# twndus/YelpRecommendation

Measured on AMD Instinct MI355X. Metric: BPR triplets/sec @ dim64, higher is better.
Workload: dtype f32; 1 GPU; BPR-MF dim=64 train step (gather+score+loss+grad+dense Adam), synthetic Yelp2018 shape; users=31668, items=38048, interactions=1566260, train_triplets_per_epoch=920629, batch_per_gpu=524288, global_batch=524288, optimizer=adam(dense), parallelism=single

## Files before the change

### include/yelprec_engine.h

```cpp
#ifndef YELPREC_ENGINE_H
#define YELPREC_ENGINE_H

#include <stdint.h>

#ifdef __cplusplus
extern "C" {
#endif

#define YR_ENGINE_VERSION 36

#define YR_ERR_UNSUPPORTED (-1)
#define YR_ERR_BADARG      (-2)

#define YR_FLAG_BAD_USER 1
#define YR_FLAG_BAD_ITEM 2

#define YR_PULL_USER_PHASE 1
#define YR_PULL_ITEM_PHASE 2

#define YR_S3REC_TRAIN 0
#define YR_S3REC_VALID 1
#define YR_S3REC_TEST  2

#define YR_OPT_ADAM  0
// ... 13 lines not shown
                float *out, int32_t *err_flag, void *stream);

int yr_mf_score_backward(const float *U, const float *I,
                         const int64_t *user, const int64_t *item, const float *gout,
                         int64_t B, int D, int64_t num_users, int64_t num_items,
                         float *gradU, float *gradI, int32_t *err_flag, void *stream);

int yr_bpr_mf_fwd_bwd(const float *U, const float *I,
                      const int64_t *user, const int64_t *pos, const int64_t *neg,
                      int64_t B, int D, int64_t num_users, int64_t num_items,
                      float inv_batch, float *gradU, float *gradI,
                      float *loss_partials, int32_t *err_flag, void *stream);

int yr_bpr_mf_scatter_step(float *U, float *I, float *gradU, float *gradI,
                           float *mU, float *vU, float *mI, float *vI, uint8_t *touched,
                           const int64_t *user, const int64_t *pos, const int64_t *neg,
                           int64_t B, int D, int64_t num_users, int64_t num_items, float inv_batch,
                           double lr, double step_size, double bc2_sqrt,
                           double beta1, double beta2, double eps, double weight_decay, int mode,
                           float *loss_partials, float *loss_out, double *loss_accum,
                           int32_t *err_flag, void *stream);
int yr_adam_dense_dual(float *p0, float *g0, float *m0, float *v0, int64_t n0,
                       float *p1, float *g1, float *m1, float *v1, int64_t n1,
                       int row_width, uint8_t *touched0, uint8_t *touched1,
                       double lr, double step_size, double bc2_sqrt,
                       double beta1, double beta2, double eps, double weight_decay, int mode,
                       const float *loss_partials, float loss_scale, float *loss_out, double *loss_accum,
                       void *stream);

int64_t yr_bpr_mf_pull_workspace_bytes(int64_t max_batch, int64_t num_users, int64_t num_items, int D);
int yr_bpr_mf_pull_step(const float *U_old, float *U_new, float *I,
                        float *mU, float *vU, float *mI, float *vI, float *gradI_out,
                        const int64_t *user, const int64_t *pos, const int64_t *neg,
                        int64_t B, int D, int64_t num_users, int64_t num_items, float inv_batch,
                        double lr, double step_size, double bc2_sqrt,
                        double beta1, double beta2, double eps, double weight_decay, int mode,
                        int deterministic, void *workspace, int64_t workspace_bytes,
                        float *loss_partials, float *loss_out, double *loss_accum,
                        int32_t *err_flag, void *stream);

int yr_bpr_mf_pull_index(const int64_t *user, const int64_t *pos, const int64_t *neg, int64_t B, int D,
                         int64_t num_users, int64_t num_items,
                         void *workspace, int64_t workspace_bytes, int32_t *err_flag, void *stream);
int yr_bpr_mf_pull_apply(const float *U_old, float *U_new, float *I,
                         float *mU, float *vU, float *mI, float *vI, float *gradI_out,
                         int64_t B, int D, int64_t num_users, int64_t num_items, float inv_batch,
                         double lr, double step_size, double bc2_sqrt,
                         double beta1, double beta2, double eps, double weight_decay, int mode,
                         int deterministic, void *workspace, int64_t workspace_bytes,
                         float *loss_partials, float *loss_out, double *loss_accum,
                         int phases, int64_t item_row_begin, int64_t item_row_end,
                         void *stream);
int yr_bpr_mf_pull_item_buckets(int64_t num_items, int D);
int yr_bpr_mf_pull_split_summary(const void *workspace, int64_t workspace_bytes, int64_t B, int D,
                                 int64_t num_users, int64_t num_items, int32_t *counters_out,
                                 int32_t *parts_out, int32_t *rule_out, void *stream);
int yr_bpr_mf_pull_apply_ordered(const float *U_old, float *U_new, float *I,
                         float *mU, float *vU, float *mI, float *vI, float *gradI_out,
                         int64_t B, int D, int64_t num_users, int64_t num_items, float inv_batch,
                         double lr, double step_size, double bc2_sqrt,
                         double beta1, double beta2, double eps, double weight_decay, int mode,
                         int deterministic, void *workspace, int64_t workspace_bytes,
                         float *loss_partials, float *loss_out, double *loss_accum,
                         int phases, int64_t item_row_begin, int64_t item_row_end,
                         const int32_t *item_bucket_order, void *stream);

#define YR_NGCF_MAX_LAYERS 8
int yr_ngcf_score_fwd(const float *const *layers, int n_layers, const int64_t *user, const int64_t *pos,
                      const int64_t *neg, int64_t B, int D, int64_t num_users, int64_t num_items,
                      float *out_pos, float *out_neg, int32_t *err_flag, void *stream);
int yr_ngcf_score_bwd(const float *const *layers, float *const *dlayers, int n_layers, const int64_t *user,
                      const int64_t *pos, const int64_t *neg, const float *gpos, const float *gneg,
                      int64_t B, int D, int64_t num_users, int64_t num_items, int32_t *err_flag, void *stream);
int yr_spmm_csr(const int32_t *rowptr, const int32_t *col, const float *val,
                const float *X, float *Y, int64_t n, int D, int accumulate,
                const int32_t *heavy_rows, int64_t n_heavy, int heavy_threshold, void *stream);
int yr_spmm_csr_sliced(const int32_t *rowptr, const int32_t *col, const float *val,
                       const float *X, float *Y, int64_t n, int D, int accumulate,
                       const int32_t *row_order, void *stream);
int yr_ngcf_dense_fwd(const float *E, const float *Z, const float *W1, const float *W2,
                      int64_t n, int D, float *Eout, void *stream);
int yr_ngcf_dense_bwd_data(const float *dEout, const float *Eout, const float *E, const float *Z,
                           const float *W1T, const float *W2T, int64_t n, int D,
                           float *dZ, float *dE, void *stream);
int yr_ngcf_dense_bwd_weight(const float *dEout, const float *Eout, const float *E, const float *Z,
                             int64_t n, int D, float *dW1, float *dW2, void *stream);

int yr_ngcf_frontier_mark(const int64_t *user, const int64_t *pos, const int64_t *neg, int64_t B,
                          int64_t num_users, int64_t num_items,
                          int32_t *flags, int32_t *rows, int32_t *count, int clear, void *stream);
int yr_ngcf_frontier_expand(const int32_t *rowptr, const int32_t *col, int64_t n,
                            const int32_t *rows_in, const int32_t *count_in, int64_t max_rows_in,
                            int32_t *flags, int32_t *rows, int32_t *count, int clear, void *stream);
int yr_spmm_csr_subset(const int32_t *rowptr, const int32_t *col, const float *val,
                       const float *X, float *Y, int64_t n, int D, int accumulate,
                       const int32_t *heavy_rows, int64_t n_heavy, int heavy_threshold,
                       const int32_t *row_active,
                       const int32_t *row_list, const int32_t *row_count, int64_t max_rows, void *stream);
int yr_spmm_csr_push_rows(const int32_t *rowptr, const int32_t *col, const float *val,
                          const float *X, float *Y, int64_t n, int D,
                          const int32_t *rows, const int32_t *count, int64_t max_rows, void *stream);
int yr_ngcf_dense_fwd_rows(const float *E, const float *Z, const float *W1, const float *W2,
                           int64_t n, int D, float *Eout,
                           const int32_t *rows, const int32_t *count, int64_t max_rows, float *zero_rows,
                           void *stream);
int yr_ngcf_dense_bwd_data_rows(const float *dEout, const float *Eout, const float *E, const float *Z,
// ... 266 lines not shown
```

### yelprecommendation_amd/_lib.py

```python
from __future__ import annotations

import ctypes as C
import os

_HERE = os.path.dirname(os.path.abspath(__file__))
LIB_PATH = os.environ.get("YR_ENGINE_LIB") or os.path.join(_HERE, "libyelprec_engine.so")
ENGINE_VERSION = 36

_p = C.c_void_p
_i64 = C.c_int64
_int = C.c_int
_f = C.c_float
_d = C.c_double

SIGNATURES = {
    "yr_engine_version": [],
    "yr_engine_arch": [],
    "yr_mf_score": [_p, _p, _p, _p, _i64, _int, _i64, _i64, _p, _p, _p],
    "yr_mf_score_backward": [_p, _p, _p, _p, _p, _i64, _int, _i64, _i64, _p, _p, _p, _p],
    "yr_bpr_mf_fwd_bwd": [_p, _p, _p, _p, _p, _i64, _int, _i64, _i64, _f, _p, _p, _p, _p, _p],
    "yr_bpr_mf_scatter_step": [_p, _p, _p, _p, _p, _p, _p, _p, _p, _p, _p, _p, _i64, _int, _i64, _i64, _f,
                               _d, _d, _d, _d, _d, _d, _d, _int, _p, _p, _p, _p, _p],
    "yr_adam_dense_dual": [_p, _p, _p, _p, _i64, _p, _p, _p, _p, _i64, _int, _p, _p,
                           _d, _d, _d, _d, _d, _d, _d, _int, _p, _f, _p, _p, _p],
# ... 4 lines not shown
    "yr_spmm_csr_sliced": [_p, _p, _p, _p, _p, _i64, _int, _int, _p, _p],
    "yr_ngcf_score_fwd": [_p, _int, _p, _p, _p, _i64, _int, _i64, _i64, _p, _p, _p, _p],
    "yr_ngcf_score_bwd": [_p, _p, _int, _p, _p, _p, _p, _p, _i64, _int, _i64, _i64, _p, _p],
    "yr_ngcf_dense_fwd": [_p, _p, _p, _p, _i64, _int, _p, _p],
    "yr_ngcf_dense_bwd_data": [_p, _p, _p, _p, _p, _p, _i64, _int, _p, _p, _p],
    "yr_ngcf_dense_bwd_weight": [_p, _p, _p, _p, _i64, _int, _p, _p, _p],
    "yr_ngcf_frontier_mark": [_p, _p, _p, _i64, _i64, _i64, _p, _p, _p, _int, _p],
    "yr_ngcf_frontier_expand": [_p, _p, _i64, _p, _p, _i64, _p, _p, _p, _int, _p],
    "yr_spmm_csr_subset": [_p, _p, _p, _p, _p, _i64, _int, _int, _p, _i64, _int, _p, _p, _p, _i64, _p],
    "yr_spmm_csr_push_rows": [_p, _p, _p, _p, _p, _i64, _int, _p, _p, _i64, _p],
    "yr_ngcf_dense_fwd_rows": [_p, _p, _p, _p, _i64, _int, _p, _p, _p, _i64, _p, _p],
    "yr_ngcf_dense_bwd_data_rows": [_p, _p, _p, _p, _p, _p, _i64, _int, _p, _p, _p, _p, _i64, _p],
    "yr_ngcf_dense_bwd_weight_rows": [_p, _p, _p, _p, _i64, _int, _p, _p, _p, _p, _i64, _p],
    "yr_ngcf_step_workspace_bytes": [_i64, _int, _int, _i64],
    "yr_ngcf_bpr_step": [_p, _p, _p, _i64, _i64, _p, _i64, _int, _i64, _p, _p, _p, _int, _int, _p, _p, _p, _i64,
                         _d, _d, _d, _d, _d, _d, _d, _int, _d, _p, _i64, _p, _p, _p, _p],
    "yr_ngcf_owned_score_workspace_bytes": [_i64, _i64],
    "yr_ngcf_owned_score_bwd": [_p, _p, _int, _p, _p, _p, _p, _p, _i64, _int, _i64, _i64, _p, _i64, _p, _p],
    "yr_ngcf_owned_dw_workspace_bytes": [_i64, _int],
    "yr_ngcf_owned_dense_bwd_weight": [_p, _p, _p, _p, _i64, _int, _p, _p, _p, _p, _i64, _p, _i64, _p],
    "yr_ngcf_frontier_order": [_p, _i64, _p, _p, _p],
    "yr_ngcf_step_ordered_workspace_bytes": [_i64, _int, _int, _i64],
    "yr_ngcf_bpr_step_ordered": [_p, _p, _p, _i64, _i64, _p, _i64, _int, _i64, _p, _p, _p, _int, _int, _p, _p, _p,
                                 _i64, _d, _d, _d, _d, _d, _d, _d, _int, _d, _p, _i64, _p, _p, _p, _p],
    "yr_gemm_f32": [_int, _int, _i64, _i64, _i64, _p, _i64, _p, _i64, _p, _i64, _p, _int, _int, _int, _p],
    "yr_gemm_f32_ex": [_int, _int, _i64, _i64, _i64, _p, _i64, _p, _i64, _p, _i64, _p, _int, _int, _int, _p, _p, _p],
    "yr_cdae_decode_loss_partials": [_i64, _i64],
    "yr_cdae_decode_loss": [_p, _p, _p, _p, _p, _i64, _i64, _int, _int, _p, _i64, _p, _p, _p, _p],
    "yr_cdae_hidden_bwd": [_p, _p, _int, _p, _i64, _int, _i64, _p, _p, _p, _p, _i64, _p, _p, _p, _int, _p],
    "yr_cdae_compact_pair": [_p, _p, _i64, _i64, C.c_uint64, _d, _p, _p, _p, _p, _p, _p, _p],
    "yr_cdae_train_lists": [_p, _p, _p, _p, _p, _i64, _i64, _i64, _int, C.c_uint64, C.c_uint64, _d, _p, _p, _p, _p, _p,
                            _p, _p, _p],
    "yr_cdae_train_lists_batched": [_p, _p, _p, _p, _p, _i64, _i64, _i64, _int, _p, _p, _i64, _d, _p, _p, _p, _p, _p,
                                    _p, _p, _p],
    "yr_cdae_loss_finalize_batched": [_p, _int, _p, _i64, _i64, _p, _p, _p, _p],
    "yr_cdae_loss_finalize": [_p, _i64, _p, _p, _p, _p],
    "yr_cdae_sampled_decode_splits": [_i64],
    "yr_cdae_sampled_decode": [_p, _p, _p, _p, _p, _p, _i64, _i64, _int, _int, _p, _p, _p, _p, _p, _p],
    "yr_cdae_hidden_init": [_p, _p, _p, _p, _i64, _int, _i64, _p, _p],
    "yr_dropout": [_p, _p, _d, _i64, _p, _p],
    "yr_sigmoid": [_p, _i64, _p],
    "yr_dropout_seeded": [_p, C.c_uint64, _d, _i64, _p, _p],
    "yr_sigmoid_bwd": [_p, _p, _p, _i64, _p],
    "yr_colsum": [_p, _i64, _i64, _p, _int, _p],
    "yr_row_scatter_add": [_p, _p, _i64, _int, _i64, _p, _p],
    "yr_nsbce_fwd": [_p, _p, _p, _i64, _p, _p, _p],
    "yr_nsbce_bwd": [_p, _p, _p, _p, _p, _i64, _p, _p],
    "yr_bpr_mf_pull_index": [_p, _p, _p, _i64, _int, _i64, _i64, _p, _i64, _p, _p],
    "yr_bpr_mf_pull_apply": [_p, _p, _p, _p, _p, _p, _p, _p, _i64, _int, _i64, _i64, _f,
                             _d, _d, _d, _d, _d, _d, _d, _int, _int, _p, _i64, _p, _p, _p, _int, _i64, _i64, _p],
    "yr_bpr_mf_pull_apply_ordered": [_p, _p, _p, _p, _p, _p, _p, _p, _i64, _int, _i64, _i64, _f,
                             _d, _d, _d, _d, _d, _d, _d, _int, _int, _p, _i64, _p, _p, _p, _int, _i64, _i64, _p, _p],
    "yr_bpr_mf_pull_item_buckets": [_i64, _int],
    "yr_bpr_mf_pull_split_summary": [_p, _i64, _i64, _int, _i64, _i64, _p, _p, _p, _p],
    "yr_loss_finalize": [_p, _f, _p, _p, _p],
    "yr_mf_scores_gemm": [_p, _p, _p, _i64, _int, _i64, _i64, _p, _i64, _p, _p],
    "yr_mf_eval_topk_planes_bytes": [_i64, _int],
    "yr_mf_eval_topk_workspace_bytes": [_i64, _i64, _int, _int, _int],
    "yr_mf_eval_topk": [_p, _p, _p, _i64, _int, _i64, _i64, _p, _p, _f, _int, _p, _p, _i64, _int, _p, _p, _p],
    "yr_mf_eval_topk_bias": [_p, _p, _p, _p, _i64, _int, _i64, _i64, _p, _p, _f, _int, _p, _p, _i64, _int, _p, _p, _p],
    "yr_ngcf_eval_topk_workspace_bytes": [_i64, _i64, _int, _int, _int],
    "yr_ngcf_eval_topk": [_p, _int, _int, _p, _i64, _i64, _i64, _p, _p, _f, _int, _p, _p, _i64, _p, _p, _p],
    "yr_topk_masked": [_p, _i64, _i64, _i64, _p, _p, _p, _f, _int, _p, _p],
    "yr_rank_metrics_workspace_bytes": [_i64],
    "yr_rank_metrics": [_p, _i64, _int, _p, _p, _p, _p, _p, _p],
    "yr_bpr_loss_fwd": [_p, _p, _i64, _p, _p],
    "yr_bpr_loss_bwd": [_p, _p, _p, _f, _i64, _p, _p, _p],
    "yr_adam_dense": [_p, _p, _p, _p, _i64, _d, _d, _d, _d, _d, _d, _d, _int, _int, _p],
    "yr_adam_dense_flat": [_p, _p, _p, _p, _p, _p, _p, _p, _p, _p, _int, _d, _d, _d, _d, _d, _d, _d, _int, _p],
    "yr_csr_rows_to_dense": [_p, _p, _p, _i64, _i64, _i64, _int, _p, _p, _p],
    "yr_negative_mask": [_p, _i64, _i64, _int, C.c_uint64, _p, _p, _p],
    "yr_sgd_dense": [_p, _p, _i64, _d, _d, _int, _p],
    "yr_cdae_sparse_part_columns": [_i64],
    "yr_cdae_compact_rows": [_p, _i64, _i64, C.c_uint64, _d, _p, _p, _p, _p],
    "yr_cdae_sparse_encode": [_p, _p, _p, _p, _p, _p, _p, _i64, _i64, _int, _i64, _int, _p, _p, _p],
    "yr_cdae_sparse_dwh": [_p, _p, _p, _p, _i64, _i64, _int, _p, _p, _p, C.c_int32, _p, _p, _p],
    "yr_cdae_sparse_encode_t": [_p, _p, _p, _p, _p, _p, _p, _i64, _i64, _int, _i64, _int, _p, _p, _p],
    "yr_cdae_sparse_dwh_t": [_p, _p, _p, _p, _i64, _i64, _int, _p, _p, _p],
    "yr_cdae_hidden_bwd_dwh_t": [_p, _p, _p, _p, _p, _int, _int, _p, _p, _i64, _i64, _int, _i64, _p, _p, _p, _p, _p, _p,
                                 _i64, _p, _p, _p],
    "yr_cdae_catalogue_bce_workspace_floats": [_i64, _i64, _int],
    "yr_cdae_catalogue_bce": [_p, _p, _p, _p, _p, _p, _i64, _i64, _i64, _int, _int, _p, _p, _p, _p, _p, _i64, _p, _p],
    "yr_cdae_owned_workspace_bytes": [_i64, _i64, _int],
    "yr_cdae_owned_decode": [_p, _p, _p, _p, _p, _p, _i64, _i64, _int, _int, _p, _p, _p, _p, _p, _p, _i64, _p],
    "yr_cdae_owned_hidden_bwd": [_p, _p, _p, _p, _p, _int, _int, _p, _p, _i64, _i64, _int, _i64, _p, _p, _p, _p, _p, _p,
                                 _i64, _p, _p, _p, _i64, _p],
    "yr_triplet_sample": [_p, _p, _i64, _p, _p, _i64, _i64, C.c_uint64, C.c_uint64, _int, _i64, _i64,
                          _p, _p, _p, _p, _p],
    "yr_dcn_assemble": [_p, _p, _p, _p, _p, _p, _int, _int, _i64, _i64, _i64, _i64, _p, _p, _p, _i64, _int, _p, _i64,
                        _p, _p],
    "yr_dcn_assemble_bwd": [_p, _i64, _p, _p, _int, _int, _i64, _i64, _i64, _i64, _p, _p, _p, _i64, _int, _p, _p, _p,
                            _p, _p, _p],
    "yr_relu_bwd": [_p, _p, _i64, _p],
    "yr_dcn_head": [_p, _i64, _p, _i64, _i64, _int, _int, _int, _p, _p, _p, _p, _int, _f, _p, _p, _p, _i64, _p, _i64,
                    _p, _p, _p, _p, _p, _p],
    "yr_dcn_score": [_p, _i64, _p, _i64, _p, _p, _p, _i64, _i64, _i64, _int, _int, _p, _p, _p, _p, _p, _p, _int, _int,
                     _p, _i64, _p, _p],
    "yr_s3rec_encode": [_p, _p, _p, _p, _i64, _int, _int, _int, _int, _i64, _int, _p, _p, _p],
    "yr_s3rec_seq_scores": [_p, _p, _p, _p, _i64, _int, _i64, _p, _p, _p, _p],
    "yr_s3rec_candidate_scores": [_p, _p, _p, _p, _i64, _i64, _int, _i64, _p, _p, _p, _p],
    "yr_s3rec_train_workspace_floats": [_i64, _int, _int, _int, _int],
    "yr_s3rec_encode_train": [_p, _p, _p, _p, _i64, _int, _int, _int, _int, _i64, C.c_uint64, _d, _p, _p, _i64, _p, _p],
    "yr_s3rec_backward": [_p, _p, _p, _i64, _int, _int, _int, _int, C.c_uint64, _d, _p, _i64, _p, _p],
    "yr_s3rec_score_grad": [_p, _p, _p, _p, _p, _i64, _int, _i64, _p, _p, _p],
    "yr_s3rec_item_grad": [_p, _p, _p, _p, _p, _p, _i64, _int, _i64, _p, _p, _p, _p],
    "yr_s3rec_catalogue_bce_workspace_floats": [_i64, _i64, _int],
# ... 61 lines not shown
```

### yelprecommendation_amd/bpr_step.py

```python
import torch

from . import engine
from .user_shard import ItemSlices, reduce_scatter_item_exchange, sharded_item_exchange


AUTO_PULL_MIN_BATCH = 24576

IMPL_NAMES = {
    "auto": "auto: atomic scatter + one Adam launch below %d triplets per rank and step, pull above" % AUTO_PULL_MIN_BATCH,
    "pull": "pull: tile partition + owner pass per table (gather/score/loss/grad/Adam fused, no atomics)",
    "atomic": "atomic: fused gather/score/loss + float-atomic scatter-add, dense Adam",
}


class BPRMFStep:
    def __init__(self, U, I, lr=1e-4, betas=(0.9, 0.999), eps=1e-8, weight_decay=0.0, optimizer="adam",
                 world_size=1, process_group=None, time_kernels=False, impl="auto", max_batch=0,
                 state=None, split_item_update=False, item_chunks=1, item_exchange="all_reduce", rank=0,
                 deterministic=False):
        if item_exchange not in ("all_reduce", "reduce_scatter"):
            raise ValueError("item_exchange must be 'all_reduce' or 'reduce_scatter'")
        width = int(U.shape[1])
        if width in engine.WIDE_WIDTHS:
            limit = max(engine.SUPPORTED_WIDTHS)
# ... 89 lines not shown
                                              self.U.device)
            self._ws_slots[slot], self._ws_batch[slot] = ws, batch
        return ws

    def step(self, u, p, n, record=False, global_batch=None, next_batch=None):
        if global_batch is None:
            global_batch = u.numel() * self.world_size
        key = self.impl_key
        if key == "auto":
            key = "pull" if (global_batch >= AUTO_PULL_MIN_BATCH * self.world_size and self._pull_ok) else "atomic"
            if self._slices is not None or self.deterministic:
                key = "pull"
        if key == "pull":
            if self._U_alt is None:
                self._U_alt = torch.empty_like(self.U)
            self.impl = IMPL_NAMES["pull"]
            self.launches = "tile_partition, owner_pass<user>, owner_pass<item>"
            return self._step_pull(u, p, n, record, global_batch, next_batch)
        if self.gU is None:
            self.gU = torch.zeros_like(self.U)
        if self.gI is None:
            self.gI = torch.zeros_like(self.I)
        self.impl = IMPL_NAMES["atomic"]
        self.launches = "bpr_fwd_bwd, adam_dual"
        return self._step_atomic(u, p, n, record, global_batch)

    def _check_triplets(self, u, p, n):
        B = u.numel()
        for name, t in (("user", u), ("pos", p), ("neg", n)):
            if not (t.is_cuda and t.dtype == torch.int64 and t.is_contiguous() and t.numel() == B):
                raise engine.EngineError(f"{name}: need a contiguous int64 GPU tensor of length {B}")
        return B

    def _build_index(self, u, p, n, slot):
        B = self._check_triplets(u, p, n)
        ws = self._workspace(B, slot)
        rc = self._lib.yr_bpr_mf_pull_index(u.data_ptr(), p.data_ptr(), n.data_ptr(), B, self.U.shape[1],
                                            self.U.shape[0], self.I.shape[0], ws.data_ptr(), ws.numel(),
                                            self._pflag, engine._stream())
        if rc:
            engine.check(rc, "yr_bpr_mf_pull_index")
        self._indexed = (slot, (u, p, n))

    def set_item_order(self, item_weight=None):
        if item_weight is None:
            self._item_order = None
            return
        nb = int(self._lib.yr_bpr_mf_pull_item_buckets(self.I.shape[0], self.I.shape[1]))
        rows = -(-self.I.shape[0] // nb) if nb else 1
        per = 1024 // self.I.shape[1]
        w = torch.zeros(nb * per, dtype=torch.float64, device=self.I.device)
        w[:self.I.shape[0]] = item_weight.to(self.I.device, torch.float64)
        load = w.view(nb, per).sum(1)
        self._item_order = torch.argsort(load, descending=True, stable=True).to(torch.int32).contiguous()

    def _auto_item_order(self, p, n):
        rows = self.I.shape[0]
        ids = torch.cat([p, n])
        ids = ids[(ids >= 0) & (ids < rows)]
        self.set_item_order(torch.bincount(ids, minlength=rows)[:rows])

    def _step_pull(self, u, p, n, record, global_batch, next_batch=None):
        B = u.numel()
        D = self.U.shape[1]
        if self._item_order is None and self.auto_item_order and B >= 4 * self.I.shape[0]:
            self._auto_item_order(p, n)
        inv = 1.0 / global_batch if global_batch else 0.0
        self.t += 1
        multi = self.world_size > 1 or self.split_item_update
        nU, nI = self.U.numel(), self.I.numel()
        alg = B * (24 + 24 * D) + 6 * 4 * (nU + (0 if multi else nI))
        ready = self._indexed is not None and all(a is b for a, b in zip(self._indexed[1], (u, p, n)))
        slot = self._indexed[0] if ready else 0

        nchunks = self.item_chunks if multi else 1
        rows = self.I.shape[0]
        gran = engine.pull_bucket_rows(D)
        bounds = [min(rows, (rows * c // nchunks + gran - 1) // gran * gran) for c in range(nchunks)] + [rows]
        both = engine.PULL_USER_PHASE | engine.PULL_ITEM_PHASE
        ploss, paccum = self.loss.data_ptr(), self.loss_accum.data_ptr()

        def apply(phases, r0, r1, with_loss=None):
            ws = self._ws_slots[slot]
            if with_loss is None:
                with_loss = bool(phases & engine.PULL_USER_PHASE)
            step_size, bc2_sqrt = engine.adam_scalars(self.t, self.lr, self.betas[0], self.betas[1])
            order = self._item_order
            rc = self._lib.yr_bpr_mf_pull_apply_ordered(
                self.U.data_ptr(), self._U_alt.data_ptr(), self._pI, self._pmU, self._pvU, self._pmI, self._pvI,
                self.gI.data_ptr() if multi else None, B, D, self.U.shape[0], rows, inv, self.lr,
                step_size, bc2_sqrt, self.betas[0], self.betas[1], self.eps, self.wd,
                engine.OPT_ADAMW if self.decoupled else engine.OPT_ADAM, 1 if self.deterministic else 0,
                ws.data_ptr(), ws.numel(), self._ppartials, ploss if with_loss else None,
                paccum if with_loss else None, phases, r0, r1, order.data_ptr() if order is not None else None,
                engine._stream())
            if rc:
                engine.check(rc, "yr_bpr_mf_pull_apply_ordered")

        def first_chunk():
            if not ready:
                self._build_index(u, p, n, slot)
            apply(both, bounds[0], bounds[1])
            if nchunks == 1:
                self._indexed = None

        def local_first():
            if record and self.time_kernels and not multi and self.t % 2 == 0:
# ... 123 lines not shown
```

### yelprecommendation_amd/csrc/bpr_pull.hip

```cpp
#include "adam.h"
#include "common.h"

namespace yr {

constexpr int kPartThreads = 1024;
#ifndef YR_ITEM_CAP
#define YR_ITEM_CAP 1024
#endif
constexpr int kCap = YR_ITEM_CAP;
constexpr int kUserCap = 768;
constexpr int kTileGroup = 256;
constexpr int kOccShift = 26;
constexpr int kOccMask = (1 << kOccShift) - 1;
constexpr int kMaxBuckets = 16383;
constexpr int kMaxOwnerGrid = 4096;
#ifndef YR_HEAVY_ROW
#define YR_HEAVY_ROW 96
#endif
constexpr int kHeavyRow = YR_HEAVY_ROW;
#ifndef YR_SPLIT_MIN
#define YR_SPLIT_MIN 2048
#endif
constexpr int kSplitMin = YR_SPLIT_MIN;
#ifndef YR_SPLIT_AVG_MIN
#define YR_SPLIT_AVG_MIN 2.5
#endif
#ifndef YR_SPLIT_AVG_TARGET
#define YR_SPLIT_AVG_TARGET 1.25
#endif
#ifndef YR_SPLIT_TARGET
#define YR_SPLIT_TARGET 1024
#endif
constexpr int kSplitTarget = YR_SPLIT_TARGET;
constexpr int kMaxParts = 64;
constexpr int kMaxTasks = 512;
constexpr int kMaxSlots = 1024;
#ifndef YR_ROWSPLIT
#define YR_ROWSPLIT 1
#endif
#ifndef YR_ROWSPLIT_MIN
#define YR_ROWSPLIT_MIN 1024
#endif
#ifndef YR_ROWSPLIT_AVG_MIN
#define YR_ROWSPLIT_AVG_MIN 2.32
#endif
#ifndef YR_ROWSPLIT_TARGET
#define YR_ROWSPLIT_TARGET 512
#endif
#ifndef YR_ROWSPLIT_AVG_TARGET
#define YR_ROWSPLIT_AVG_TARGET 1.16
#endif
constexpr int kRowSplitMin = YR_ROWSPLIT_MIN;
constexpr int kRowSplitTarget = YR_ROWSPLIT_TARGET;
constexpr int kMaxRowTasks = YR_ROWSPLIT ? 512 : 0;
constexpr int kBuildLanes = 4;
#ifndef YR_DEAL
#define YR_DEAL 1
#endif
#ifndef YR_DEAL_MIN
#define YR_DEAL_MIN 256
#endif
constexpr int kDealMin = YR_DEAL_MIN;
#ifndef YR_OWNER_WAVES
#define YR_OWNER_WAVES 8
#endif
#ifndef YR_USER_UNROLL
#define YR_USER_UNROLL 1
#endif
#ifndef YR_ITEM_UNROLL
#define YR_ITEM_UNROLL 2
#endif
constexpr int kUserUnroll = YR_USER_UNROLL;
constexpr int kItemUnroll = YR_ITEM_UNROLL;

struct PullAdam {
  AdamScalars c;
  int decoupled;
};

__device__ __forceinline__ float4 ld4o(const float* base, uint32_t off) {
  return *reinterpret_cast<const float4*>(reinterpret_cast<const char*>(base) + (uint32_t)(off * 4u));
}

template <int D>
struct PullGeom {
  static_assert(D == 16 || D == 32 || D == 64 || D == 128, "unsupported width");
  static constexpr int LPR = D / 4;
  static constexpr int GPW = kWave / LPR;
// ... 92 lines not shown
  const int total = s_cnt[nb];
  if (side == 0) {
#pragma unroll
    for (int k = 0; k < PT; ++k)
      if (u[k] >= 0) {
        const int b = tile * TILE + k * kPartThreads + tid;
        s_stage[s_cnt[u[k] >> shift] + ra[k]] = make_int4(p[k], n[k], b, u[k] & rmask);
      }
    if (bad && err_flag) atomicOr(err_flag, bad);
    __syncthreads();
    int4* out = rec + (int64_t)tile * TILE;
    for (int i = tid; i < total; i += kPartThreads) out[i] = s_stage[i];
  } else {
    int2* stage2 = reinterpret_cast<int2*>(s_stage);
#pragma unroll
    for (int k = 0; k < PT; ++k)
      if (u[k] >= 0) {
        const int b = tile * TILE + k * kPartThreads + tid;
        stage2[s_cnt[p[k] >> shift] + ra[k]] = make_int2(u[k] | ((p[k] & rmask) << kOccShift), b);
        stage2[s_cnt[n[k] >> shift] + rb[k]] = make_int2(u[k] | ((n[k] & rmask) << kOccShift), b | (int)0x80000000);
      }
    __syncthreads();
    int4* out = reinterpret_cast<int4*>(occ + (int64_t)tile * TILE * 2);
    const int n16 = (total + 1) >> 1;
    for (int i = tid; i < n16; i += kPartThreads) out[i] = s_stage[i];
  }
}

#ifdef YR_STAMPS
__device__ long long g_stamps[8192 * 8];
__device__ int g_walk_iters[8192 * 4];
#define YR_STAMP(i) do { if (threadIdx.x == 0 && first_bucket) g_stamps[(blockIdx.x + (USER ? 0 : 4096)) * 8 + (i)] = wall_clock64(); } while (0)
#else
#define YR_STAMP(i)
#endif

struct OwnerArgs {
  const float* own_old;
  float* own_new;
  const float* other;
  float* m;
  float* v;
  float* grad_out;
  const int32_t* off;
  const void* recs;
  float* coeff;
  float* loss_partials;
  float* loss_out;
  double* loss_accum;
  int finalize;
  int nb, T, tile_stride;
  int rows;
  int bucket_begin, bucket_end;
  const int32_t* order;
  int heavy_t;
  float inv_batch;
  PullAdam adam;
  char* split;
  float* scratch;
  const int32_t* b_off;
  int helper_blocks, build_blocks, b_nb;
  int b_split_min, b_split_target;
  int b_rowsplit_min, b_rowsplit_quad;
};

__host__ __device__ __forceinline__ size_t split_per(int nbI) { return ((size_t)nbI * 4 + 15) & ~(size_t)15; }
__device__ __forceinline__ int32_t* split_counters(char* b) { return (int32_t*)b; }
__device__ __forceinline__ int32_t* split_parts(char* b) { return (int32_t*)(b + 16); }
__device__ __forceinline__ int32_t* split_slot(char* b, int nbI) { return (int32_t*)(b + 16 + split_per(nbI)); }
__device__ __forceinline__ int32_t* split_arrive(char* b, int nbI) { return (int32_t*)(b + 16 + 2 * split_per(nbI)); }
__device__ __forceinline__ int4* split_tasks(char* b, int nbI) { return (int4*)(b + 16 + 3 * split_per(nbI)); }
__device__ __forceinline__ int2* split_row_tasks(char* b, int nbI) { return (int2*)(split_tasks(b, nbI) + kMaxTasks); }

__device__ __forceinline__ void build_splits(const OwnerArgs& a, int builder) {
  const int k = (builder * kBlock + (int)threadIdx.x) / kBuildLanes, j = threadIdx.x % kBuildLanes;
  int total = 0;
  if (k < a.b_nb) {
    int t = j;
    const int64_t pitch = a.b_nb + 1;
    for (; t + 3 * kBuildLanes < a.T; t += 4 * kBuildLanes) {
      const int32_t* o0 = a.b_off + (int64_t)t * pitch + k;
      const int32_t* o1 = o0 + kBuildLanes * pitch;
      const int32_t* o2 = o1 + kBuildLanes * pitch;
      const int32_t* o3 = o2 + kBuildLanes * pitch;
      const int a0 = o0[0], b0 = o0[1], a1 = o1[0], b1 = o1[1], a2 = o2[0], b2 = o2[1], a3 = o3[0], b3 = o3[1];
      total += ((b0 - a0) + (b1 - a1)) + ((b2 - a2) + (b3 - a3));
    }
    for (; t < a.T; t += kBuildLanes) {
      const int32_t* orow = a.b_off + (int64_t)t * (a.b_nb + 1) + k;
      total += orow[1] - orow[0];
    }
  }
#pragma unroll
  for (int m = 1; m < kBuildLanes; m <<= 1) total += __shfl_xor(total, m, kWave);
  if (k >= a.b_nb || j != 0) return;
  int parts = 1;
  if (total >= a.b_split_min) {
    parts = (total + a.b_split_target - 1) / a.b_split_target;
    parts = min(parts, min(kMaxParts, a.T));
  }
  int slot = 0;
  if (parts > 1) {
    slot = atomicAdd(split_counters(a.split) + 1, parts);
    const int first = atomicAdd(split_counters(a.split), parts - 1);
    const bool fits = slot + parts <= kMaxSlots && first + parts - 1 <= kMaxTasks;
    for (int q = 1; q < parts; ++q)
// ... 340 lines not shown
  constexpr int D = F::D, R = F::R;
  __threadfence();
  float4 acc = zero4();
  if (finisher) {
    for (int q = 0; q < parts; ++q) {
      const float4 p = ld4(slots + (int64_t)q * (R * D) + row_t * D + lc);
      acc.x += p.x; acc.y += p.y; acc.z += p.z; acc.w += p.w;
    }
  }
  return acc;
}

template <int D, bool USER, bool FUSE_ADAM, bool DET, int RPWX = 0>
__global__ __launch_bounds__(kBlock, YR_OWNER_WAVES) void owner_pass_kernel(OwnerArgs a) {
  using F = OwnerForm<D, USER, FUSE_ADAM, DET, RPWX>;
  constexpr int LPR = F::LPR, GPW = F::GPW, RPW = F::RPW, R = F::R, DEAL_BAR = F::DEAL_BAR, CAP = F::CAP, PT = F::PT;
  constexpr bool DEAL = F::DEAL, TAG_SLOT = F::TAG_SLOT, LOOKUP = F::LOOKUP;
  __shared__ int s_pre[kTileGroup + 1];
  __shared__ int s_base[kTileGroup];
  __shared__ int s_cnt[kWave];
  __shared__ int s_start[kWave];
  __shared__ int s_light[kWave + 1];
  __shared__ unsigned char s_slotof[DEAL ? kWave : 1];
  __shared__ unsigned char s_rowof[DEAL ? kWave : 1];
  __shared__ int s_x[CAP];
  __shared__ int s_y[CAP];
  __shared__ int s_z[(USER || DET) ? CAP : 1];
  __shared__ unsigned short s_idx[CAP];
  __shared__ float4 s_own[USER ? R * LPR : 1];
  __shared__ float4 s_heavy[kWavesPerBlock][LPR];
  __shared__ float s_red[kWavesPerBlock];
  __shared__ int s_scan[kWavesPerBlock];
  __shared__ int s_n;
  const int tid = threadIdx.x, lane = tid & (kWave - 1), wave = tid / kWave;
  const int grp = lane / LPR, l = lane % LPR;
  const bool finisher = grp < RPW;
  const int row_l = wave * RPW + (finisher ? grp : 0);
  float loss = 0.0f;
  __shared__ int s_last;
  const OwnerLds s = {s_pre, s_base, s_cnt, s_start, s_rowof, s_x, s_y, s_z, s_idx, s_scan, &s_n, &s_last};
  if (USER && (int)blockIdx.x < a.build_blocks) {
    build_splits(a, blockIdx.x);
    return;
  }
  const int hb = USER ? a.build_blocks : a.helper_blocks;
  const bool helper = !USER && (int)blockIdx.x < hb;
  const int owners = (int)gridDim.x - hb;
#ifdef YR_STAMPS
  bool first_bucket = true;
  int walk_iters = 0, heavy_iters = 0;
#endif
  YR_STAMP(0);

  for (int ks = helper ? (int)blockIdx.x : a.bucket_begin + (int)blockIdx.x - hb;
       helper ? ks == (int)blockIdx.x : ks < a.bucket_end; ks += owners) {
    int k, part = 0, parts = 1;
    int4 cnt = make_int4(0, 0, 0, 0);
    if (!USER && a.split) cnt = *reinterpret_cast<const int4*>(a.split);
    int k_own = ks;
    if (!helper && a.order) k_own = a.order[ks];
    const int c_tasks = __builtin_amdgcn_readfirstlane(cnt.x), c_slots = __builtin_amdgcn_readfirstlane(cnt.y);
    const int c_rows = __builtin_amdgcn_readfirstlane(cnt.z);
    const bool pools_hold = USER || !a.split || (c_tasks <= kMaxTasks && c_slots <= kMaxSlots);
    const int tile_tasks = (USER || !a.split || !pools_hold) ? 0 : c_tasks;
    const bool rows_hold = !USER && YR_ROWSPLIT && a.split && c_rows <= kMaxRowTasks && tile_tasks + c_rows <= kMaxTasks;
    const bool row_helper = YR_ROWSPLIT && helper && ks >= tile_tasks;
    if (row_helper) {
      const int j = kMaxTasks - 1 - ks;
      if (!rows_hold || j >= c_rows) break;
      const int2 task = split_row_tasks(a.split, a.nb)[j];
      k = __builtin_amdgcn_readfirstlane(task.x);
      part = __builtin_amdgcn_readfirstlane(task.y);
      if (k < a.bucket_begin || k >= a.bucket_end) break;
    } else if (helper) {
      if (ks >= tile_tasks) break;
      const int4 task = split_tasks(a.split, a.nb)[ks];
      k = __builtin_amdgcn_readfirstlane(task.x);
      part = __builtin_amdgcn_readfirstlane(task.y);
      if (k < a.bucket_begin || k >= a.bucket_end) break;
    } else {
      k = __builtin_amdgcn_readfirstlane(k_own);
    }
    if (!USER && a.split) {
      const int word = __builtin_amdgcn_readfirstlane(split_parts(a.split)[k]);
      if (word > 1 && pools_hold) parts = word;
      if (YR_ROWSPLIT && word < 0 && rows_hold) parts = word;
    }
    if (row_helper && parts >= 0) break;
    const int t_begin = parts < 0 ? 0 : __builtin_amdgcn_readfirstlane(a.T * part / parts);
    const int t_end = parts < 0 ? a.T : __builtin_amdgcn_readfirstlane(a.T * (part + 1) / parts);
    int row_t = row_l;
    int row_f = k * R + row_t;
    bool valid_f = finisher && row_f < a.rows && (USER || row_kept(row_t, part, parts));
    uint32_t o_f = (uint32_t)(row_f * D + 4 * l);
    bool bound = false;
    if (USER && finisher) s_own[row_l * LPR + l] = valid_f ? ld4o(a.own_old, o_f) : zero4();
    YR_STAMP(1);
    RowSums<LPR, GPW> sums;
    sums.clear();

    for (int tg0 = t_begin; tg0 < t_end; tg0 += kTileGroup) {
      const int nt = min(kTileGroup, t_end - tg0);
      const int total = scan_segments(a, s, tid, k, tg0, nt);
      YR_STAMP(2);

      for (int c0 = 0, cend = 0, sub = 0; c0 < total; c0 = cend) {
        cend = min(total, c0 + CAP);
        int wt = 0;
        bool windowed = false;
        if (DET) windowed = cut_chunk_at_tiles<CAP>(s_pre, nt, c0, total, cend, wt);
        if (tid < kWave) s_cnt[tid] = 0;
        if (DET && tid == 0) s_n = 0;
        __syncthreads();
        int key[PT];
        int n_rec = cend - c0;
        if (DET && windowed) {
          n_rec = load_window<F>(a, s, tid, part, parts, tg0, wt, c0, sub, cend, key);
          if (n_rec == 0) {
            __syncthreads();
            continue;
          }
        } else {
        uint32_t addr[PT];
#pragma unroll
        for (int q = 0; q < PT; ++q) {
          const int j = c0 + tid + q * kBlock;
          key[q] = j < cend ? 0 : -1;
          int tlo = 0, thi = nt;
          while (thi - tlo > 1) {
            const int mid = (tlo + thi) >> 1;
            if (s_pre[mid] <= j) tlo = mid; else thi = mid;
          }
          addr[q] = j < cend ? (uint32_t)(s_base[tlo] + (j - s_pre[tlo])) : 0u;
        }
// ... 285 lines not shown
  const int rc = pull_check_common(B, D, num_users, num_items, workspace, workspace_bytes);
  if (rc) return rc;
  if (B == 0) return 0;
  if (!user || !pos || !neg) return YR_ERR_BADARG;
  const PullPlan p = make_plan(B, num_users, num_items, D, false);
  char* w = static_cast<char*>(workspace);
  int32_t* offU = (int32_t*)(w + p.o_offU);
  int32_t* offI = (int32_t*)(w + p.o_offI);
  int4* rec = (int4*)(w + p.o_rec);
  int2* occ = (int2*)(w + p.o_occ);
  const int stage_off = (((p.nbU > p.nbI ? p.nbU : p.nbI) + 1) + 3) & ~3;
  const size_t lds = (size_t)stage_off * 4 + (size_t)p.tile * 16;
  const dim3 grid(p.T, 2);
  hipStream_t s = (hipStream_t)stream;
#define YR_PART_CASE(PT)                                                                                         \
  case PT: {                                                                                                     \
    static bool raised = false;                    \
    if (!raised && lds > 65536) {                                                                                \
      const hipError_t e = hipFuncSetAttribute(reinterpret_cast<const void*>(&tile_partition_kernel<PT>),        \
                                               hipFuncAttributeMaxDynamicSharedMemorySize, 160 * 1024 - 256);    \
      if (e != hipSuccess) return (int)e;                                                                        \
      raised = true;                                                                                             \
    }                                                                                                            \
    hipLaunchKernelGGL((tile_partition_kernel<PT>), grid, dim3(kPartThreads), lds, s, user, pos, neg, B, num_users, \
                       num_items, p.shiftU, p.shiftI, p.nbU, p.nbI, offU, offI, rec, occ, err_flag, stage_off,   \
                       (int32_t*)(w + p.o_split));                                                              \
  } break
  switch (p.pt) {
    YR_PART_CASE(1);
    YR_PART_CASE(2);
    YR_PART_CASE(4);
    default: return YR_ERR_BADARG;
  }
#undef YR_PART_CASE
  return launch_status();
}

template <int D>
static int pull_apply_impl(const float* U_old, float* U_new, float* I, float* mU, float* vU, float* mI, float* vI,
                           float* gradI_out, int64_t B, int64_t nU, int64_t nI, float inv_batch, const PullAdam& adam,
                           int deterministic, void* workspace, float* loss_partials, float* loss_out,
                           double* loss_accum, int phases, int64_t item_begin, int64_t item_end,
                           const int32_t* item_order, hipStream_t s) {
  const PullPlan p = make_plan(B, nU, nI, D, false);
  char* w = static_cast<char*>(workspace);
  const bool want_loss = loss_out || loss_accum;
  if (phases & YR_PULL_USER_PHASE) {
    OwnerArgs ua{};
    ua.own_old = U_old; ua.own_new = U_new; ua.other = I; ua.m = mU; ua.v = vU; ua.grad_out = nullptr;
    ua.off = (const int32_t*)(w + p.o_offU); ua.recs = w + p.o_rec; ua.coeff = (float*)(w + p.o_coeff);
    ua.loss_partials = loss_partials;
    ua.nb = p.nbU; ua.T = p.T; ua.tile_stride = p.tile; ua.rows = (int)nU;
    ua.bucket_begin = 0; ua.bucket_end = p.nbU;
    ua.order = nullptr;
    ua.heavy_t = kHeavyRow; ua.inv_batch = inv_batch; ua.adam = adam;
    ua.build_blocks = (p.nbI * kBuildLanes + kBlock - 1) / kBlock;
    ua.b_off = (const int32_t*)(w + p.o_offI); ua.b_nb = p.nbI;
    const SplitRule rule = split_rule(B, p.nbI, D);
    ua.b_split_min = rule.split_min; ua.b_split_target = rule.split_target;
    ua.b_rowsplit_min = rule.row_min; ua.b_rowsplit_quad = rule.row_quad;
    ua.split = w + p.o_split;
    const int gu = (p.nbU < YR_LOSS_PARTIALS ? p.nbU : YR_LOSS_PARTIALS) + ua.build_blocks;
    if (p.narrow_users && deterministic)
      hipLaunchKernelGGL((owner_pass_kernel<D, true, true, true, 1>), dim3(gu), dim3(kBlock), 0, s, ua);
    else if (p.narrow_users)
      hipLaunchKernelGGL((owner_pass_kernel<D, true, true, false, 1>), dim3(gu), dim3(kBlock), 0, s, ua);
    else if (deterministic)
      hipLaunchKernelGGL((owner_pass_kernel<D, true, true, true>), dim3(gu), dim3(kBlock), 0, s, ua);
    else
      hipLaunchKernelGGL((owner_pass_kernel<D, true, true, false>), dim3(gu), dim3(kBlock), 0, s, ua);
  }
  const bool items = (phases & YR_PULL_ITEM_PHASE) && item_end > item_begin;
  if (items) {
    OwnerArgs ia{};
    ia.own_old = I; ia.own_new = I; ia.other = U_old; ia.m = mI; ia.v = vI; ia.grad_out = gradI_out;
    ia.off = (const int32_t*)(w + p.o_offI); ia.recs = w + p.o_occ; ia.coeff = (float*)(w + p.o_coeff);
    ia.loss_partials = loss_partials; ia.loss_out = loss_out; ia.loss_accum = loss_accum;
    ia.finalize = want_loss ? 1 : 0;
    ia.nb = p.nbI; ia.T = p.T; ia.tile_stride = 2 * p.tile; ia.rows = (int)nI;
    ia.bucket_begin = (int)(item_begin >> p.shiftI);
    ia.bucket_end = (int)((item_end + (1 << p.shiftI) - 1) >> p.shiftI);
    ia.order = (item_order && ia.bucket_begin == 0 && ia.bucket_end == p.nbI) ? item_order : nullptr;
    ia.heavy_t = kHeavyRow; ia.inv_batch = inv_batch; ia.adam = adam;
    ia.helper_blocks = kMaxTasks;
    ia.split = w + p.o_split;
    ia.scratch = (float*)(w + p.o_scratch);
    int gi = ia.bucket_end - ia.bucket_begin;
    if (gi > kMaxOwnerGrid) gi = kMaxOwnerGrid;
    gi += ia.helper_blocks;
    if (gradI_out && deterministic)
      hipLaunchKernelGGL((owner_pass_kernel<D, false, false, true>), dim3(gi), dim3(kBlock), 0, s, ia);
    else if (gradI_out)
      hipLaunchKernelGGL((owner_pass_kernel<D, false, false, false>), dim3(gi), dim3(kBlock), 0, s, ia);
    else if (deterministic)
      hipLaunchKernelGGL((owner_pass_kernel<D, false, true, true>), dim3(gi), dim3(kBlock), 0, s, ia);
    else
      hipLaunchKernelGGL((owner_pass_kernel<D, false, true, false>), dim3(gi), dim3(kBlock), 0, s, ia);
  } else if (want_loss) {
    hipLaunchKernelGGL(pull_loss_finalize_kernel, dim3(1), dim3(kBlock), 0, s, loss_partials, inv_batch, loss_out,
                       loss_accum);
  }
  return launch_status();
}

extern "C" int yr_bpr_mf_pull_item_buckets(int64_t num_items, int D) {
  if (num_items <= 0 || (D != 16 && D != 32 && D != 64 && D != 128)) return YR_ERR_BADARG;
  const int sh = bucket_shift(D);
  return (int)((num_items + (1 << sh) - 1) >> sh);
}

extern "C" int yr_bpr_mf_pull_split_summary(const void* workspace, int64_t workspace_bytes, int64_t B, int D,
                                            int64_t num_users, int64_t num_items, int32_t* counters_out,
                                            int32_t* parts_out, int32_t* rule_out, void* stream) {
  if (!rule_out || B <= 0 || num_users <= 0 || num_items <= 0) return YR_ERR_BADARG;
  if (D != 16 && D != 32 && D != 64 && D != 128) return YR_ERR_UNSUPPORTED;
  const PullPlan p = make_plan(B, num_users, num_items, D, false);
  const SplitRule r = split_rule(B, p.nbI, D);
  const int32_t rule[8] = {r.split_min, r.split_target, r.row_min, r.row_target, r.row_quad, r.row_max_parts,
                           kMaxRowTasks, YR_ROWSPLIT};
  for (int i = 0; i < 8; ++i) rule_out[i] = rule[i];
  if (!workspace) return (counters_out || parts_out) ? YR_ERR_BADARG : 0;
  const int rc = pull_check_common(B, D, num_users, num_items, workspace, workspace_bytes);
  if (rc) return rc;
  const char* blk = static_cast<const char*>(workspace) + p.o_split;
  hipStream_t s = (hipStream_t)stream;
  hipError_t e = hipSuccess;
  if (counters_out) e = hipMemcpyAsync(counters_out, blk, 16, hipMemcpyDeviceToHost, s);
  if (e == hipSuccess && parts_out)
    e = hipMemcpyAsync(parts_out, blk + 16, (size_t)p.nbI * 4, hipMemcpyDeviceToHost, s);
  if (e == hipSuccess) e = hipStreamSynchronize(s);
  return (int)e;
}

extern "C" int yr_bpr_mf_pull_apply_ordered(const float* U_old, float* U_new, float* I, float* mU, float* vU,
                                            float* mI, float* vI, float* gradI_out, int64_t B, int D,
                                            int64_t num_users, int64_t num_items, float inv_batch, double lr,
                                            double step_size, double bc2_sqrt, double beta1, double beta2, double eps,
                                            double weight_decay, int mode, int deterministic, void* workspace,
                                            int64_t workspace_bytes, float* loss_partials, float* loss_out,
                                            double* loss_accum, int phases, int64_t item_row_begin,
                                            int64_t item_row_end, const int32_t* item_bucket_order, void* stream) {
  int rc = pull_check_common(B, D, num_users, num_items, workspace, workspace_bytes);
  if (rc) return rc;
  if (!(phases & (YR_PULL_USER_PHASE | YR_PULL_ITEM_PHASE))) return YR_ERR_BADARG;
  if (item_row_begin < 0 || item_row_end > num_items || item_row_begin > item_row_end) return YR_ERR_BADARG;
  const int R = 1 << bucket_shift(D);
  if (item_row_begin % R != 0 || (item_row_end % R != 0 && item_row_end != num_items)) return YR_ERR_BADARG;
  if (!U_old || !U_new || U_old == U_new || !I || !mU || !vU || !loss_partials) return YR_ERR_BADARG;
  if (!gradI_out && (!mI || !vI)) return YR_ERR_BADARG;
  if (mode != YR_OPT_ADAM && mode != YR_OPT_ADAMW) return YR_ERR_UNSUPPORTED;
  const PullAdam c = {adam_scalars(lr, step_size, bc2_sqrt, beta1, beta2, eps, weight_decay), mode == YR_OPT_ADAMW};
  hipStream_t s = (hipStream_t)stream;
#define YR_APPLY_CASE(DD)                                                                                       \
  case DD:                                                                                                      \
    return pull_apply_impl<DD>(U_old, U_new, I, mU, vU, mI, vI, gradI_out, B, num_users, num_items, inv_batch,  \
                               c, deterministic ? 1 : 0, workspace, loss_partials, loss_out, loss_accum, phases,      \
                               item_row_begin, item_row_end, item_bucket_order, s)
  switch (D) {
    YR_APPLY_CASE(16);
    YR_APPLY_CASE(32);
    YR_APPLY_CASE(64);
// ... 38 lines not shown
```

Measured before the change: 5.054 billion triplets/s.

## Place owner buckets so XCD-interleaved blocks own contiguous row runs

Introduces an owner slot to bucket mapping that groups runs of adjacent buckets onto the same XCD, given that workgroups are dispatched round-robin across 8 XCDs. Neighbouring rows then share an L2. The item start order is now computed on the host and is XCD-class aware, so heavy buckets stay on their home XCD while load is still balanced. The grid is padded to whole rounds, and padded slots beyond the bucket range skip their work. This aims to improve L2 locality for the embedding, Adam state and record reads, at the cost of extra idle slots and a host-side sort.

```diff
diff --git a/include/yelprec_engine.h b/include/yelprec_engine.h
--- a/include/yelprec_engine.h
+++ b/include/yelprec_engine.h
@@ -89,6 +89,8 @@
                          int phases, int64_t item_row_begin, int64_t item_row_end,
                          void *stream);
 int yr_bpr_mf_pull_item_buckets(int64_t num_items, int D);
+int yr_bpr_mf_pull_owner_bucket(int slot, int nb);
+int yr_bpr_mf_pull_item_start_order(const double *bucket_load_host, int nb, int32_t *order_out);
 int yr_bpr_mf_pull_split_summary(const void *workspace, int64_t workspace_bytes, int64_t B, int D,
                                  int64_t num_users, int64_t num_items, int32_t *counters_out,
                                  int32_t *parts_out, int32_t *rule_out, void *stream);
diff --git a/yelprecommendation_amd/_lib.py b/yelprecommendation_amd/_lib.py
--- a/yelprecommendation_amd/_lib.py
+++ b/yelprecommendation_amd/_lib.py
@@ -80,6 +80,8 @@
     "yr_bpr_mf_pull_apply_ordered": [_p, _p, _p, _p, _p, _p, _p, _p, _i64, _int, _i64, _i64, _f,
                              _d, _d, _d, _d, _d, _d, _d, _int, _int, _p, _i64, _p, _p, _p, _int, _i64, _i64, _p, _p],
     "yr_bpr_mf_pull_item_buckets": [_i64, _int],
+    "yr_bpr_mf_pull_owner_bucket": [_int, _int],
+    "yr_bpr_mf_pull_item_start_order": [_p, _int, _p],
     "yr_bpr_mf_pull_split_summary": [_p, _i64, _i64, _int, _i64, _i64, _p, _p, _p, _p],
     "yr_loss_finalize": [_p, _f, _p, _p, _p],
     "yr_mf_scores_gemm": [_p, _p, _p, _i64, _int, _i64, _i64, _p, _i64, _p, _p],
diff --git a/yelprecommendation_amd/bpr_step.py b/yelprecommendation_amd/bpr_step.py
--- a/yelprecommendation_amd/bpr_step.py
+++ b/yelprecommendation_amd/bpr_step.py
@@ -165,7 +165,11 @@
         w = torch.zeros(nb * per, dtype=torch.float64, device=self.I.device)
         w[:self.I.shape[0]] = item_weight.to(self.I.device, torch.float64)
         load = w.view(nb, per).sum(1)
-        self._item_order = torch.argsort(load, descending=True, stable=True).to(torch.int32).contiguous()
+        load = load.cpu().contiguous()
+        order = torch.empty(nb, dtype=torch.int32)
+        engine.check(self._lib.yr_bpr_mf_pull_item_start_order(load.data_ptr(), nb, order.data_ptr()),
+                     "yr_bpr_mf_pull_item_start_order")
+        self._item_order = order.to(self.I.device)
 
     def _auto_item_order(self, p, n):
         rows = self.I.shape[0]
diff --git a/yelprecommendation_amd/csrc/bpr_pull.hip b/yelprecommendation_amd/csrc/bpr_pull.hip
--- a/yelprecommendation_amd/csrc/bpr_pull.hip
+++ b/yelprecommendation_amd/csrc/bpr_pull.hip
@@ -1,5 +1,6 @@
 #include "adam.h"
 #include "common.h"
+#include "pull_placement.h"
 
 namespace yr {
 
@@ -14,6 +15,8 @@
 constexpr int kOccMask = (1 << kOccShift) - 1;
 constexpr int kMaxBuckets = 16383;
 constexpr int kMaxOwnerGrid = 4096;
+static_assert(kMaxOwnerGrid % kXcdRound == 0 && YR_LOSS_PARTIALS % kXcdRound == 0,
+              "a capped grid strides by whole rounds of runs: ks += owners keeps owner_bucket a bijection");
 #ifndef YR_HEAVY_ROW
 #define YR_HEAVY_ROW 96
 #endif
@@ -34,6 +37,7 @@
 constexpr int kSplitTarget = YR_SPLIT_TARGET;
 constexpr int kMaxParts = 64;
 constexpr int kMaxTasks = 512;
+static_assert(kMaxTasks % 8 == 0, "the owners behind the helpers keep slot % 8 == blockIdx.x % 8 (owner_bucket)");
 constexpr int kMaxSlots = 1024;
 #ifndef YR_ROWSPLIT
 #define YR_ROWSPLIT 1
@@ -232,6 +236,7 @@
   int nb, T, tile_stride;
   int rows;
   int bucket_begin, bucket_end;
+  int slots;
   const int32_t* order;
   int heavy_t;
   float inv_batch;
@@ -678,12 +683,12 @@
 #endif
   YR_STAMP(0);
 
-  for (int ks = helper ? (int)blockIdx.x : a.bucket_begin + (int)blockIdx.x - hb;
-       helper ? ks == (int)blockIdx.x : ks < a.bucket_end; ks += owners) {
+  for (int ks = helper ? (int)blockIdx.x : (int)blockIdx.x - hb;
+       helper ? ks == (int)blockIdx.x : ks < a.slots; ks += owners) {
     int k, part = 0, parts = 1;
     int4 cnt = make_int4(0, 0, 0, 0);
     if (!USER && a.split) cnt = *reinterpret_cast<const int4*>(a.split);
-    int k_own = ks;
+    int k_own = a.bucket_begin + owner_bucket(ks);
     if (!helper && a.order) k_own = a.order[ks];
     const int c_tasks = __builtin_amdgcn_readfirstlane(cnt.x), c_slots = __builtin_amdgcn_readfirstlane(cnt.y);
     const int c_rows = __builtin_amdgcn_readfirstlane(cnt.z);
@@ -706,6 +711,7 @@
       if (k < a.bucket_begin || k >= a.bucket_end) break;
     } else {
       k = __builtin_amdgcn_readfirstlane(k_own);
+      if (k >= a.bucket_end) continue;
     }
     if (!USER && a.split) {
       const int word = __builtin_amdgcn_readfirstlane(split_parts(a.split)[k]);
@@ -1097,6 +1103,7 @@
     ua.loss_partials = loss_partials;
     ua.nb = p.nbU; ua.T = p.T; ua.tile_stride = p.tile; ua.rows = (int)nU;
     ua.bucket_begin = 0; ua.bucket_end = p.nbU;
+    ua.slots = owner_slots(p.nbU);
     ua.order = nullptr;
     ua.heavy_t = kHeavyRow; ua.inv_batch = inv_batch; ua.adam = adam;
     ua.build_blocks = (p.nbI * kBuildLanes + kBlock - 1) / kBlock;
@@ -1105,7 +1112,7 @@
     ua.b_split_min = rule.split_min; ua.b_split_target = rule.split_target;
     ua.b_rowsplit_min = rule.row_min; ua.b_rowsplit_quad = rule.row_quad;
     ua.split = w + p.o_split;
-    const int gu = (p.nbU < YR_LOSS_PARTIALS ? p.nbU : YR_LOSS_PARTIALS) + ua.build_blocks;
+    const int gu = (ua.slots < YR_LOSS_PARTIALS ? ua.slots : YR_LOSS_PARTIALS) + ua.build_blocks;
     if (p.narrow_users && deterministic)
       hipLaunchKernelGGL((owner_pass_kernel<D, true, true, true, 1>), dim3(gu), dim3(kBlock), 0, s, ua);
     else if (p.narrow_users)
@@ -1126,11 +1133,12 @@
     ia.bucket_begin = (int)(item_begin >> p.shiftI);
     ia.bucket_end = (int)((item_end + (1 << p.shiftI) - 1) >> p.shiftI);
     ia.order = (item_order && ia.bucket_begin == 0 && ia.bucket_end == p.nbI) ? item_order : nullptr;
+    ia.slots = ia.order ? ia.bucket_end : owner_slots(ia.bucket_end - ia.bucket_begin);
     ia.heavy_t = kHeavyRow; ia.inv_batch = inv_batch; ia.adam = adam;
     ia.helper_blocks = kMaxTasks;
-    ia.split = w + p.o_split;
+    ia.split = B > 0 ? w + p.o_split : nullptr;
     ia.scratch = (float*)(w + p.o_scratch);
-    int gi = ia.bucket_end - ia.bucket_begin;
+    int gi = ia.slots;
     if (gi > kMaxOwnerGrid) gi = kMaxOwnerGrid;
     gi += ia.helper_blocks;
     if (gradI_out && deterministic)
@@ -1152,6 +1160,20 @@
   if (num_items <= 0 || (D != 16 && D != 32 && D != 64 && D != 128)) return YR_ERR_BADARG;
   const int sh = bucket_shift(D);
   return (int)((num_items + (1 << sh) - 1) >> sh);
+}
+
+extern "C" int yr_bpr_mf_pull_owner_bucket(int slot, int nb) {
+  if (nb <= 0 || nb > kMaxBuckets || slot < 0 || slot >= owner_slots(nb)) return YR_ERR_BADARG;
+  const int k = owner_bucket(slot);
+  return k < nb ? k : -1;
+}
+
+extern "C" int yr_bpr_mf_pull_item_start_order(const double* bucket_load_host, int nb, int32_t* order_out) {
+  if (!bucket_load_host || !order_out || nb <= 0 || nb > kMaxBuckets) return YR_ERR_BADARG;
+  for (int k = 0; k < nb; ++k)
+    if (!(bucket_load_host[k] == bucket_load_host[k])) return YR_ERR_BADARG;
+  owner_start_order(bucket_load_host, nb, order_out);
+  return 0;
 }
 
 extern "C" int yr_bpr_mf_pull_split_summary(const void* workspace, int64_t workspace_bytes, int64_t B, int D,
diff --git a/yelprecommendation_amd/csrc/pull_placement.h b/yelprecommendation_amd/csrc/pull_placement.h
--- /dev/null
+++ b/yelprecommendation_amd/csrc/pull_placement.h
@@ -0,0 +1,56 @@
+#pragma once
+#include <algorithm>
+#include <cstdint>
+#include <vector>
+
+#if defined(__HIPCC__) || defined(__CUDACC__)
+#define YR_PLACEMENT_FN __host__ __device__ __forceinline__
+#else
+#define YR_PLACEMENT_FN inline
+#endif
+
+#ifndef YR_XCD_RUN
+#define YR_XCD_RUN 8
+#endif
+
+namespace yr {
+
+constexpr int kXcds = 8;
+constexpr int kXcdRun = YR_XCD_RUN;
+static_assert(kXcdRun >= 1 && kXcdRun <= 256 && (kXcdRun & (kXcdRun - 1)) == 0, "runs of a power of two buckets");
+constexpr int kXcdRunShift = __builtin_ctz(kXcdRun);
+constexpr int kXcdRound = kXcds * kXcdRun;
+
+YR_PLACEMENT_FN int owner_slots(int n) { return (n + kXcdRound - 1) & ~(kXcdRound - 1); }
+
+YR_PLACEMENT_FN int owner_bucket(int s) {
+  const int c = s & (kXcds - 1), j = s >> 3;
+  return ((((j >> kXcdRunShift) << 3) + c) << kXcdRunShift) + (j & (kXcdRun - 1));
+}
+
+inline void owner_start_order(const double* load, int nb, int32_t* order) {
+  std::vector<int32_t> by_load(nb);
+  for (int k = 0; k < nb; ++k) by_load[k] = k;
+  std::stable_sort(by_load.begin(), by_load.end(), [load](int32_t a, int32_t b) { return load[a] > load[b]; });
+  std::vector<unsigned char> cls(nb), used(nb, 0);
+  for (int s = 0, n = owner_slots(nb); s < n; ++s)
+    if (owner_bucket(s) < nb) cls[owner_bucket(s)] = (unsigned char)(s & (kXcds - 1));
+  std::vector<int32_t> queue[kXcds];
+  for (int i = 0; i < nb; ++i) queue[cls[by_load[i]]].push_back(by_load[i]);
+  size_t head[kXcds] = {}, rest = 0;
+  for (int s = 0; s < nb; ++s) {
+    const int c = s & (kXcds - 1);
+    while (head[c] < queue[c].size() && used[queue[c][head[c]]]) ++head[c];
+    int32_t k;
+    if (head[c] < queue[c].size()) {
+      k = queue[c][head[c]++];
+    } else {
+      while (used[by_load[rest]]) ++rest;
+      k = by_load[rest];
+    }
+    used[k] = 1;
+    order[s] = k;
+  }
+}
+
+}
```

Measured after the change: 5.226 billion triplets/s, median of 6. 3.4% higher.
